# diaoenmao/Multimodal-Controller-for-Generative-Models

Hardware: AMD Instinct MI355X
Metric: images/sec (train step) MCGAN CIFAR-10 32x32 (higher is better)
Workload: dtype bf16

## Files before the change

### include/mcgen_hip.h

```cpp
#ifndef MCGEN_HIP_H
#define MCGEN_HIP_H

#include <stdint.h>

#ifdef __cplusplus
extern "C" {
#endif

enum { MCGEN_F32 = 0, MCGEN_BF16 = 1 };

const char* mcgen_last_error(void);
int mcgen_abi_version(void);

typedef struct {
    const void*  x;
    const float* scale;
    const float* shift;
    const float* code;
    const int16_t* cmap;
    int32_t C;
    int32_t ups;
    int32_t relu;
    int32_t ksize;
    int32_t group_n;
// ... 361 lines not shown
int mcgen_cvae_enc_dembed(const float* part, const float* w, float* de, int N, int H, int C, int Cin, int Cimg, int E,
                          void* stream);
int mcgen_cvae_latent_fwd(const void* ml, int ldm, const float* eps, const float* w, const int64_t* label, float* mu,
                          float* logvar, void* zrow, float* kl, float* kld, int dtype, int N, int L, int E, int M, int Cp,
                          void* stream);
int mcgen_cvae_latent_bwd(const void* dzrow, int ldz, const float* mu, const float* logvar, const float* eps, float inv_numel,
                          void* dml, float* de, int dtype, int N, int L, int E, int Cq, void* stream);

int mcgen_cglow_prior(const float* b_p, const float* s_p, const float* w_e, const float* b_e, const float* s_e,
                      const int64_t* label, void* out, int dtype, int N, int HW, int C2, int M, int Cp, void* stream);
int mcgen_cglow_prior_bwd(const void* dprior, const float* b_p, const float* s_p, const float* w_e, const float* b_e,
                          const float* s_e, const int64_t* label, float* workspace, float* db_p, float* ds_p, float* dw_p,
                          int64_t dw_p_elems, float* dw_e, float* db_e, float* ds_e, int dtype, int N, int HW, int C2, int M,
                          int Cp, void* stream);

#ifdef __cplusplus
}
#endif
#endif
```

### multimodal-controller-for-generative-models_amd/csrc/small_ops.hip

```cpp
#include "mcgen_common.h"
#include <string.h>

static thread_local char g_err[512] = "";
int mcgen_fail(const char* fmt, ...) {
    va_list ap; va_start(ap, fmt); vsnprintf(g_err, sizeof(g_err), fmt, ap); va_end(ap);
    return 1;
}
extern "C" const char* mcgen_last_error(void) { return g_err; }
extern "C" int mcgen_abi_version(void) { return 9; }

namespace {

inline int grid_for(size_t n, int block = 256, int cap = 4096) {
    size_t b = (n + block - 1) / block; if (b < 1) b = 1; if (b > (size_t)cap) b = cap; return (int)b;
}
#define STREAM(s) reinterpret_cast<hipStream_t>(s)

template <typename T> __device__ __forceinline__ float ldf(const T* p) { return Elem<T>::to_f(*p); }

template <typename T>
__global__ void nchw_to_nhwc_kernel(const float* __restrict__ src, T* __restrict__ dst, int N, int C, int HW, int Cp) {
    const size_t total = (size_t)N * HW * Cp;
    for (size_t i = blockIdx.x * (size_t)blockDim.x + threadIdx.x; i < total; i += (size_t)gridDim.x * blockDim.x) {
        const int c = (int)(i % Cp); const size_t pix = i / Cp;
// ... 100 lines not shown
__device__ __forceinline__ void prep_weight_body(const mcgen_prep_t& d, const float* __restrict__ sigma_base) {
    const int KS = d.ksize, Cout = d.Cout, Cin = d.Cin, transpose = d.transpose, row_perm = d.row_perm;
    const float* __restrict__ w = d.w;
    T* __restrict__ img = reinterpret_cast<T*>(d.image);
    const int ntap = KS * KS;
    if (d.layout == 1) {
        const int cow = (Cout + 15) / 16 * 16, krows = (Cin + 7) / 8 * 8 + 1;
        const size_t totalk = (size_t)ntap * krows * cow;
        const float sck = (d.sigma_idx >= 0) ? d.wscale / sigma_base[d.sigma_idx] : d.wscale;
        for (size_t i = blockIdx.x * (size_t)blockDim.x + threadIdx.x; i < totalk; i += (size_t)gridDim.x * blockDim.x) {
            const int co = (int)(i % cow); size_t t = i / cow;
            const int k = (int)(t % krows); const int tap = (int)(t / krows);
            float v = 0.f;
            if (co < Cout && k < Cin) v = w[((size_t)co * Cin + k) * ntap + tap] * sck;
            img[i] = Elem<T>::from_f(v);
        }
        return;
    }
    const int16_t* __restrict__ kmap = transpose ? nullptr : d.kmap;
    const int rows = transpose ? Cin : Cout, kdim = kmap ? d.kcount : (transpose ? Cout : Cin);
    const int rows_w = (rows + 15) / 16 * 16;
    const int nchunk = (((kdim + 7) / 8 * 8) + MCGEN_CK - 1) / MCGEN_CK;
    const float sc = (d.sigma_idx >= 0) ? d.wscale / sigma_base[d.sigma_idx] : d.wscale;
    const int16_t* __restrict__ rmap = transpose ? nullptr : d.rmap;
    __shared__ __attribute__((aligned(16))) T stage[9][8 * MCGEN_CK];
    const int rgroups = rows_w / 8;
    const int groups = nchunk * rgroups;
    const int r8 = threadIdx.x >> 5, col = threadIdx.x & 31;
    constexpr int UPT = 8 * MCGEN_CK * (int)sizeof(T) / 16;
    for (int gi = blockIdx.x; gi < groups; gi += gridDim.x) {
// ... 1509 lines not shown
```

### multimodal-controller-for-generative-models_amd/gan_engine.py

```python
from __future__ import annotations

from typing import Dict, List, Optional

import torch
import torch.nn as nn

from . import ops
from ._tuning import flag as _flag
from .ops import Seg

Tensor = torch.Tensor


def _bump(t: Tensor):
    torch.autograd.graph.increment_version(t)


class FlatState:

    def __init__(self, tensors: List[Tensor]):
        self.tensors = tensors
        self.flat: Optional[Tensor] = None
        self.offsets: List[int] = []
        self._index = {id(t): i for i, t in enumerate(tensors)}
# ... 48 lines not shown
_PM_MAX_MODES = 16
class Nhwc:
    __slots__ = ('t', 'c')

    def __init__(self, t: Tensor, c: int):
        self.t, self.c = t, c

    @property
    def shape(self):
        n, h, w, _ = self.t.shape
        return torch.Size((n, self.c, h, w))


_SN_SNAP = _flag('MCGEN_SN_SNAP', '1') != '0'
_D0_FUSE = _flag('MCGEN_D0_FUSE', '1') != '0'
_BN_PAR = _flag('MCGEN_BN_PAR', '1') != '0'
_pending_counters: Dict[int, List[Tensor]] = {}
_pending_running: List = []


def _flush_counters():
    for k, ts in _pending_counters.items():
        if ts:
            torch._foreach_add_(ts, k)
    _pending_counters.clear()
    if _pending_running:
        ops.bn_running_batch(_pending_running)
        _pending_running.clear()


# ... 486 lines not shown
        red.__exit__(None, None, None)
        yield (0, off_cut if (cut > 0 and _BUCKETS and split) else gflat.numel(), True)


class _SNConv:

    def __init__(self, module: nn.Module, idx: int):
        self.m = module
        self.idx = idx
        w = module.weight_orig
        self.cout, self.cin = w.shape[0], w.shape[1]
        self.ks = w.shape[2] if w.dim() == 4 else 1


class DiscriminatorEngine:
    def __init__(self, dis, dtype: torch.dtype = torch.float32):
        self.dis = dis
        self.dtype = dtype
        blocks = list(dis.blocks.children())
        self.res = [b for b in blocks if hasattr(b, 'mc_1')]
        t = len(self.res)
        self.tail_mc, self.tail_lin = blocks[t + 1], blocks[t + 3].module
        self.sn: List[_SNConv] = []
        for m in dis.modules():
            if hasattr(m, 'weight_orig'):
                self.sn.append(_SNConv(m, len(self.sn)))
        self.sn_of = {s.m: s for s in self.sn}
        params = list(dis.parameters())
        sn_w = {id(s.m.weight_orig) for s in self.sn}
        self.plain = [p for p in params if id(p) not in sn_w]
# ... 35 lines not shown
            self.img[name] = t
            return t

        def cat(name, a: _SNConv, b: _SNConv, transpose):
            na = ops.weight_image_elems(a.cout, a.cin, a.ks, transpose)
            nb = ops.weight_image_elems(b.cout, b.cin, b.ks, transpose)
            t = torch.empty(na + nb, dtype=dt, device=dev)
            self.img[name] = t
            return t[:na], t[na:]

        fwd, bwd = [], []
        W = lambda s: s.m.weight_orig.detach()
        b0 = self.res[0]
        c1m, c2m, scm = (self.sn_of[b0.conv[0].module], self.sn_of[b0.conv[3].module], self.sn_of[b0.shortcut[0].module])
        fwd.append((W(c1m), img('0.c1', c1m, False), False, 1, c1m.idx, 1.0))
        if _D0_FUSE:
            ta, tb = cat('0.c2s', c2m, scm, False)
            fwd += [(W(c2m), ta, False, 1, c2m.idx, 1.0), (W(scm), tb, False, 1, scm.idx, 1.0)]
        else:
            fwd += [(W(scm), img('0.sc', scm, False), False, 1, scm.idx, 1.0),
                    (W(c2m), img('0.c2', c2m, False), False, 1, c2m.idx, 1.0)]
        bwd.append((W(c2m), img('0.c2t', c2m, True), True, 1, c2m.idx, 0.25))
        ta, tb = cat('0.dimg', c1m, scm, True)
        bwd += [(W(c1m), ta, True, 1, c1m.idx, 1.0), (W(scm), tb, True, 1, scm.idx, 0.25)]
        for i, b in enumerate(self.res[1:], start=1):
            c1m, c2m = self.sn_of[b.conv[2].module], self.sn_of[b.conv[5].module]
            has_sc, pooled = len(b.shortcut) > 0, len(b.conv) == 7
            a = 0.25 if pooled else 1.0
            fwd.append((W(c1m), img(f'{i}.c1', c1m, False), False, 1, c1m.idx, 1.0))
            if has_sc:
                scm = self.sn_of[b.shortcut[1].module]
                ta, tb = cat(f'{i}.c2s', c2m, scm, False)
                fwd += [(W(c2m), ta, False, 1, c2m.idx, 1.0), (W(scm), tb, False, 1, scm.idx, 1.0)]
                bwd.append((W(scm), img(f'{i}.sct', scm, True), True, 1, scm.idx, a))
            else:
                fwd.append((W(c2m), img(f'{i}.c2', c2m, False), False, 1, c2m.idx, 1.0))
            bwd += [(W(c2m), img(f'{i}.c2t', c2m, True), True, 1, c2m.idx, a),
                    (W(c1m), img(f'{i}.c1t', c1m, True), True, 1, c1m.idx, 1.0)]
        self._prep_fwd, self._prep_bwd = ops.PrepBatch(fwd, dt), ops.PrepBatch(bwd, dt)
        self._prep_all = ops.PrepBatch(fwd + bwd, dt)
        self._bwd_sigma = None

    def _ensure_preps(self):
        if self._prep_fwd is None or self._prep_fwd.dtype != self.dtype or not self._prep_fwd.valid():
            self._build_preps()

    def _power_iters(self, rounds: int, train: bool):
        fp, fuv = self._ensure_flat()
        nsn = len(self.sn)
        if train and _SN_ROUNDS and not _SN_FUSED and rounds >= int(_flag('MCGEN_SN_ROUNDS_MIN', '1')):
            sigma, snap = ops.sn_power_iter_rounds(fp, fuv, self._layers_dev, nsn, rounds,
                                                   max(s.cout for s in self.sn), max(s.cin * s.ks * s.ks for s in self.sn))
            for s in self.sn:
                _bump(s.m.weight_u); _bump(s.m.weight_v)
            self._sn_ratio = sigma[rounds] if rounds >= 2 else None
            return [(sigma[r], snap[r]) for r in range(rounds)]
        self._sn_ratio = None
        if not _SN_FUSED:
            out = []
# ... 66 lines not shown
            uses = [(None, c1m.idx), (None, scm.idx), (0, c2m.idx)]
            for i, b in enumerate(self.res[1:], start=1):
                c1m, c2m = self.sn_of[b.conv[2].module], self.sn_of[b.conv[5].module]
                uses += [(2 * i - 1, c1m.idx), (2 * i, c2m.idx)]
                if len(b.shortcut) > 0:
                    uses.append((2 * i - 1, self.sn_of[b.shortcut[1].module].idx))
            uses.append((len(self._codes.mcs) - 1, self.sn_of[self.tail_lin].idx))
            self._uses = uses
            self._use_idx = {}
        return self._uses

    def _forward_body(self, x_nchw: Tensor, ctx, code_of, tail_loss: Optional[str] = None):
        dt = self.dtype
        n = x_nchw.shape[0]
        sigma = ctx['sigma']
        self._ensure_preps()
        prep = self._prep_all if ctx.get('train', True) else self._prep_fwd
        job = ctx.pop('codes_job', None)
        if job is not None:
            cb, label, reps, scale, n_half, sink = job
            sink(ops.prep_and_codes(prep, sigma, cb, label, reps, scale, n_half))
        else:
            prep.run(sigma)
        if ctx.get('train', True):
            self._bwd_sigma = sigma
        I = self.img
        img = x_nchw.t if isinstance(x_nchw, Nhwc) else ops.to_nhwc(x_nchw.detach().contiguous(), dt)
        if img.dtype != dt:
            raise RuntimeError(f'Nhwc input is {img.dtype}, the engine computes in {dt}')
        ctx['img'], ctx['nhwc'] = img, isinstance(x_nchw, Nhwc)
        b0 = self.res[0]
        c1m, c2m, scm = (self.sn_of[b0.conv[0].module], self.sn_of[b0.conv[3].module], self.sn_of[b0.shortcut[0].module])
        co = c1m.cout
        c1, _ = ops.conv_fused([Seg(img, code=code_of(None, c1m.idx))], I['0.c1'], co, bias=c1m.m.bias)
        code = code_of(0, c2m.idx)
        if _D0_FUSE:
            y, _ = ops.conv_fused([Seg(c1, code=code, relu=True), Seg(img, ksize=1, code=code_of(None, scm.idx))], I['0.c2s'], co,
                                  bias=c2m.m.bias, bias2=scm.m.bias, pool=True, alpha=0.25)
        else:
            sc, _ = ops.conv_fused([Seg(img, ksize=1, code=code_of(None, scm.idx))], I['0.sc'], co, bias=scm.m.bias, pool=True, alpha=0.25)
            y, _ = ops.conv_fused([Seg(c1, code=code, relu=True)], I['0.c2'], co, bias=c2m.m.bias, pool=True, alpha=0.25, res=sc)
        ctx['blocks'].append({'c1': c1, 'code': code})
        x = y
        for i, b in enumerate(self.res[1:], start=1):
            c1m, c2m = self.sn_of[b.conv[2].module], self.sn_of[b.conv[5].module]
            has_sc = len(b.shortcut) > 0
            pooled = len(b.conv) == 7
            code1, code2 = code_of(2 * i - 1, c1m.idx), code_of(2 * i, c2m.idx)
            code1s = None
            c1, _ = ops.conv_fused([Seg(x, code=code1, relu=True)], I[f'{i}.c1'], c1m.cout, bias=c1m.m.bias)
            if has_sc:
                scm = self.sn_of[b.shortcut[1].module]
                code1s = code_of(2 * i - 1, scm.idx)
# ... 152 lines not shown
                dy, _ = ops.conv_fused([Seg(dc1)], I[f'{bi}.c1t'], c1m.cin, ocode=code1, gate_x=x, res=res)
                if want_w and bi == cut and _BUCKETS and split:
                    red.__exit__(None, None, None)
                    fix(bk['hi'], bk['i_cut'])
                    if _BUCKETS and split:
                        yield (bk['off_cut'], fp.numel(), False)
                    red = ops.deferred_reduces()
                    red.__enter__()
            b0, bc = self.res[0], ctx['blocks'][0]
            c1m, c2m, scm = (self.sn_of[b0.conv[0].module], self.sn_of[b0.conv[3].module], self.sn_of[b0.shortcut[0].module])
            c1, code, img = bc['c1'], bc['code'], ctx['img']
            if want_w:
                wgrad_all(lambda sl: Seg(c1[sl], code=U(0, sl), relu=True), dy, c2m.cout, c2m.cin, c2m.m.weight_orig,
                          c2m.m.bias, scm.m.bias, dy_ups=True, alpha=0.25)
                wgrad_all(lambda sl: Seg(img[sl], ksize=1), dy, scm.cout, scm.cin, scm.m.weight_orig, dy_ups=True, alpha=0.25)
            dc1, _ = ops.conv_fused([Seg(dy, ups=True)], I['0.c2t'], c2m.cin, ocode=code, gate_x=c1)
            if want_w:
                wgrad_all(lambda sl: Seg(img[sl]), dc1, c1m.cout, c1m.cin, c1m.m.weight_orig, c1m.m.bias)
            dimg = None
            if need_input_grad:
                if pair is not None:
                    raise RuntimeError('input gradients of a paired pass are not needed by the D update and not built')
                dimg_t, _ = ops.conv_fused([Seg(dc1), Seg(dy, ksize=1, ups=True)], I['0.dimg'], c1m.cin, cy=img.shape[-1])
                dimg = Nhwc(dimg_t, c1m.cin) if ctx.get('nhwc') else ops.to_nchw(dimg_t, c1m.cin)
        except BaseException as e:
            red.__exit__(type(e), e, None)
            raise
        red.__exit__(None, None, None)
        if want_w:
            if defer_fix and pair is not None and not (_BUCKETS and split) and not accumulate:
                self.pending_fix = {'g0': passes[0][1], 'g1': passes[1][1], 'uv0': uv, 'uv1': pair['uv2'], 'sigma0': sigma,
# ... 8 lines not shown
```

### multimodal-controller-for-generative-models_amd/ops.py

```python
from __future__ import annotations

import ctypes as C
import os as _os
from dataclasses import dataclass
from typing import NamedTuple, Optional, Sequence, Tuple

import torch

from . import _lib
from ._lib import check
from ._tuning import flag as _flag

Tensor = torch.Tensor


def _dt(dtype: torch.dtype) -> int:
    if dtype == torch.float32:
        return _lib.F32
    if dtype == torch.bfloat16:
        return _lib.BF16
    raise _lib.McgenError(f'unsupported compute dtype {dtype}')


def _stream() -> int:
# ... 251 lines not shown
    cout, cin = w.shape[0], w.shape[1]
    ks = w.shape[2] if w.dim() == 4 else 1
    n = weight_image_k_elems(cout, cin, ks)
    if out is None:
        out = torch.empty(n, dtype=dtype, device=w.device)
    assert out.numel() == n and out.dtype == dtype
    check(_lib.load().mcgen_prep_weight_k(_f32(w.contiguous()), _p(out), _dt(dtype), cout, cin, ks, _f32(sigma), float(wscale), _stream()),
          'prep_weight_k')
    return out


def weight_image_elems(cout: int, cin: int, ksize: int, transpose: bool = False) -> int:
    return int(_lib.load().mcgen_weight_image_elems(cout, cin, ksize, int(transpose)))


def prep_weight(w: Tensor, dtype: torch.dtype, transpose: bool = False, row_perm: int = 1,
                sigma: Optional[Tensor] = None, wscale: float = 1.0, out: Optional[Tensor] = None) -> Tensor:
    cout, cin = w.shape[0], w.shape[1]
    ks = w.shape[2] if w.dim() == 4 else 1
    n = weight_image_elems(cout, cin, ks, transpose)
    if out is None:
        out = torch.empty(n, dtype=dtype, device=w.device)
    assert out.numel() == n and out.dtype == dtype
    check(_lib.load().mcgen_prep_weight(_f32(w), _p(out), _dt(dtype), cout, cin, ks, int(transpose), row_perm,
                                        _f32(sigma), float(wscale), _stream()), 'prep_weight')
    return out


def conv_fused(segs: Sequence[Seg], wimg: Tensor, cout: int, *, bias: Optional[Tensor] = None, bias2: Optional[Tensor] = None,
               pool: bool = False, alpha: float = 1.0, res: Optional[Tensor] = None,
               ocode: Optional[Tensor] = None, gate_x: Optional[Tensor] = None,
               gscale: Optional[Tensor] = None, gshift: Optional[Tensor] = None,
               gmean: Optional[Tensor] = None, grstd: Optional[Tensor] = None,
               tanh: bool = False, stats_mode: int = 0, cy: Optional[int] = None,
               out: Optional[Tensor] = None, kmajor: int = 0, ycmap: Optional[Tensor] = None,
               y_group: int = 0, wsel: Optional[Tensor] = None, order: Optional[Tensor] = None,
               yperm: Optional[Tensor] = None) -> Tuple[Tensor, Optional[Tensor]]:
    s0 = segs[0]
    n = s0.x.shape[0]
    h = s0.x.shape[1] * (2 if s0.ups else 1)
    w = s0.x.shape[2] * (2 if s0.ups else 1)
    dtype = s0.x.dtype
    cy = cy or pad8(cout)
    ho, wo = (h // 2, w // 2) if pool else (h, w)
    p = _lib.Conv()
    p.nseg = len(segs)
    for i, s in enumerate(segs):
        if s.x.dtype != dtype:
            raise _lib.McgenError('all segments must share the compute dtype')
        hs = s.x.shape[1] * (2 if s.ups else 1)
        if hs != h or s.x.shape[0] != n:
            raise _lib.McgenError('segments disagree on the convolution resolution')
        s.fill(p.seg[i])
    if wimg.dtype != dtype:
        raise _lib.McgenError(f'weight image dtype {wimg.dtype} != activation dtype {dtype}')
    if kmajor:
        need = sum(s.ksize * s.ksize * ((s.cw or s.x.shape[-1]) + 1) for s in segs) * pad16(cout)
    else:
        need = sum(((s.x.shape[-1] + 31) // 32) * s.ksize * s.ksize for s in segs) * pad16(cout) * 32
    if wsel is not None:
        if wsel.dtype != torch.int32 or wsel.numel() != n or (order is not None and (order.dtype != torch.int32 or order.numel() != n)):
            raise _lib.McgenError('wsel / order must be int32 [N]')
        if wimg.numel() % need:
            raise _lib.McgenError(f'weight sets: {wimg.numel()} elements are not a multiple of one image ({need})')
    elif order is not None:
        raise _lib.McgenError('order comes with wsel')
    elif wimg.numel() != need:
        raise _lib.McgenError(f'weight image has {wimg.numel()} elements, the segments need {need}')
    y = out if out is not None else torch.empty((n, ho, wo, cy), dtype=dtype, device=s0.x.device)
    if y_group:
        if out is None or tuple(y.shape) != (2 * n, ho, wo, cy) or y.dtype != dtype or not y.is_contiguous():
# ... 21 lines not shown
        if wsel is None or yperm.dtype != torch.int16 or yperm.dim() != 2 or yperm.shape[0] * need != wimg.numel() or not yperm.is_contiguous():
            raise _lib.McgenError('yperm must be a contiguous int16 [sets, stride] table that comes with wsel')
        p.yperm, p.yperm_stride = _p(yperm), yperm.shape[1]
    p.ycmap, p.ycmap_stride = None, 0
    if ycmap is not None:
        if ycmap.dtype != torch.int16 or tuple(ycmap.shape) != (n, cmap_stride(pad8(cout))):
            raise _lib.McgenError(f'ycmap must be int16 {(n, cmap_stride(pad8(cout)))}')
        p.ycmap, p.ycmap_stride = _p(ycmap), ycmap.shape[1]
    stats = None
    lib = _lib.load()
    plan = _conv_plan(p, dtype)
    if stats_mode:
        stats = torch.empty((plan.m_tiles, 2, pad16(cout) if (ycmap is not None or yperm is not None) else cy), dtype=torch.float32, device=y.device)
        p.stats = _p(stats)
    kflops = 2.0 * n * h * w * cout * sum(s.ksize * s.ksize * s.x.shape[-1] for s in segs)

    def _name():
        base = f'conv_fused<{"bf16" if dtype == torch.bfloat16 else "f32"},{plan.bm},{plan.bn}{(",mc", ",gk")[kmajor - 1] if kmajor else ""}>'
        if plan.form:
            base = ('conv_skinny<bf16>', 'conv_smap<bf16>', 'conv_px1<bf16>', 'conv_c8<bf16>', 'conv_head<bf16>')[plan.form - 1]
        if _PROF_SHAPES:
            base += f' N{n} {h}x{w} ' + '+'.join(f'{s.x.shape[-1]}k{s.ksize}' for s in segs) + f'->{cout}' + \
                ('g' if gate_x is not None else '') + ('p' if pool else '') + (f's{stats_mode}' if stats_mode else '')
        return base
    if TILE_LOG is not None:
        bm, bn = C.c_int(plan.bm), C.c_int(plan.bn)
        if plan.form:
            check(lib.mcgen_conv_tile(C.byref(p), _dt(dtype), C.byref(bm), C.byref(bn)), 'conv_tile')
        TILE_LOG.append((bm.value, bn.value))
    if FORM_LOG is not None:
        FORM_LOG.append(kmajor)
    if KERNEL_LOG is not None:
        KERNEL_LOG.append(int(plan.form))
    _timed(_name, kflops, lambda: check(lib.mcgen_conv_fused(C.byref(p), _dt(dtype), _stream()), 'conv_fused'),
           lambda: _nbytes(wimg, y, res, gate_x, *[s.x for s in segs]))
    return y, stats


MULTI_LOG = None
WGRAD_LOG = None
BATCH_LOG = None
_deferred = None
_MULTI = _flag('MCGEN_WGRAD_MULTI', '1') != '0'
_BATCH = _flag('MCGEN_WGRAD_BATCH', '1') != '0'
_WG_GROUP_MIN = 1 << 30 if _flag('MCGEN_WGRAD_GROUP', '1') == '0' else 4
_WG_MAX_SPLITS = int(_flag('MCGEN_WGRAD_MAX_SPLITS', '128'))
_WG_TARGET = int(_flag('MCGEN_WGRAD_TARGET', '256'))
_WG_W1 = float(_flag('MCGEN_WG_W1', '0.55'))
_WG_FIX = float(_flag('MCGEN_WG_FIX', '5'))
# ... 506 lines not shown
                                 weight_decay, _p(step), _stream()), 'adam')


def _struct_table(arr, device) -> Tensor:
    return torch.frombuffer(bytearray(bytes(arr)), dtype=torch.uint8).to(device)


class PrepBatch:

    def __init__(self, jobs, dtype: torch.dtype):
        self.dtype = dtype
        self.jobs = jobs
        arr = (_lib.Prep * len(jobs))()
        for d, job in zip(arr, jobs):
            w, img, transpose, row_perm, sidx, wscale = job[:6]
            kmajor = bool(job[6]) if len(job) > 6 else False
            kmap, kcount = (job[7], int(job[8])) if len(job) > 8 and job[7] is not None else (None, 0)
            rmap = job[9] if len(job) > 9 else None
            cout, cin = w.shape[0], w.shape[1]
            ks = w.shape[2] if w.dim() == 4 else 1
            if kmap is not None:
                assert not kmajor and not transpose and row_perm == 1 and kmap.dtype == torch.int16 and kmap.numel() >= kcount
                want = weight_image_elems(cout, kcount, ks, False)
            else:
                want = weight_image_k_elems(cout, cin, ks) if kmajor else weight_image_elems(cout, cin, ks, transpose)
            assert img.numel() == want and img.dtype == dtype and not (kmajor and (transpose or row_perm != 1))
            d.w, d.image = _f32(w), _p(img)
            d.Cout, d.Cin, d.ksize, d.transpose, d.row_perm, d.sigma_idx = cout, cin, ks, int(transpose), row_perm, sidx
            d.wscale, d.layout = float(wscale), int(kmajor)
            d.kmap, d.kcount = _p(kmap), kcount
            if rmap is not None:
                assert not kmajor and not transpose and row_perm == 1 and rmap.dtype == torch.int16 and rmap.numel() >= cout and rmap.is_contiguous()
            d.rmap = _p(rmap)
        self.key = tuple((w.data_ptr(), img.data_ptr()) for w, img, *_ in jobs)
        self.table = _struct_table(arr, jobs[0][0].device)
        self.n = len(jobs)

    def valid(self) -> bool:
        return self.key == tuple((w.data_ptr(), img.data_ptr()) for w, img, *_ in self.jobs)

    def run(self, sigma: Optional[Tensor] = None):
        check(_lib.load().mcgen_prep_weight_batch(_p(self.table), self.n, _f32(sigma), _dt(self.dtype), _stream()),
              'prep_weight_batch')

# ... 810 lines not shown
```

Baseline: 17750.

## Add folded 4x4 kernels for discriminator block0 pooled conv and its backward

Adds specialized HIP kernels for the first discriminator residual block at 32x32. The forward kernel folds the 3x3 conv plus 2x2 average pool into a 16-tap stride-2 conv with the 1x1 shortcut fused in. The backward kernel folds the upsample plus transposed 3x3 conv into four phase-wise 2x2 convs. Both use LDS windows, an async weight ring fed by global_load_lds, and MFMA. New weight-image layouts (2 and 3) are prepared for them, so the pool and upsample no longer waste FLOPs on a full-resolution conv. The cost is a narrow shape guard, a large LDS footprint with one block per CU, and extra prep work.

```diff
diff --git a/include/mcgen_hip.h b/include/mcgen_hip.h
--- a/include/mcgen_hip.h
+++ b/include/mcgen_hip.h
@@ -399,6 +399,13 @@
                           int64_t dw_p_elems, float* dw_e, float* db_e, float* ds_e, int dtype, int N, int HW, int C2, int M,
                           int Cp, void* stream);
 
+int mcgen_conv_fold_fwd_ok(const mcgen_conv_t* p, int dtype);
+int mcgen_conv_fold_fwd(const mcgen_conv_t* p, int dtype, void* stream);
+int mcgen_conv_fold_bwd_ok(const mcgen_conv_t* p, int dtype);
+int mcgen_conv_fold_bwd(const mcgen_conv_t* p, int dtype, void* stream);
+int mcgen_conv_fold_bn(const mcgen_conv_t* p);
+int64_t mcgen_fold_image_elems(int Cout, int Cin, int transpose, int shortcut);
+
 #ifdef __cplusplus
 }
 #endif
diff --git a/multimodal-controller-for-generative-models_amd/csrc/conv_fold.hip b/multimodal-controller-for-generative-models_amd/csrc/conv_fold.hip
--- /dev/null
+++ b/multimodal-controller-for-generative-models_amd/csrc/conv_fold.hip
@@ -0,0 +1,382 @@
+#include "conv_tile.h"
+
+namespace {
+
+constexpr int FD_NT = 512;
+constexpr int FD_WN = 2, FD_FM = 4;
+constexpr int FD_BROW = MCGEN_CK * 2;
+constexpr int FD_RB = 3, FD_DIST = 2;
+constexpr int FD_AP = 96;
+constexpr int FD_COLS = 17, FD_ROWS = 34;
+constexpr int FD_PLANE = FD_ROWS * FD_COLS * FD_AP;
+constexpr int FD_WIN = 2 * FD_PLANE;
+constexpr int FD_TAPS = 16;
+constexpr int FB_PIX = 18 * 18, FB_PB = 256;
+constexpr int FB_WIN = FB_PIX * FB_PB;
+
+template <int BN> struct FdCfg {
+    static constexpr int FN = BN / FD_WN / 16;
+    static constexpr int SLOT = BN * FD_BROW, KB = SLOT / 1024, RING = FD_RB * SLOT;
+    static constexpr int EP = BN + 4;
+    static constexpr int CH = BN / 8, PROWS = FD_NT / CH;
+    static constexpr int FWD_EPI = 256 * EP * 4;
+    static constexpr int FWD_LDS = (FD_WIN + RING) > FWD_EPI ? (FD_WIN + RING) : FWD_EPI;
+    static constexpr int BWD_EPI = 64 * EP * 4;
+    static constexpr int BWD_LDS = FB_WIN + RING + BWD_EPI;
+    static_assert(FWD_LDS <= 160 * 1024 && BWD_LDS <= 160 * 1024, "LDS");
+};
+
+template <int BN>
+struct FdRing {
+    using G = FdCfg<BN>;
+    int d_src;
+    int w_row_off[G::FN];
+    __device__ __forceinline__ void setup(int wave, int lane, int wn, int row0) {
+        const int row = wave * 16 + (lane >> 2), pu = lane & 3;
+        d_src = (row0 + row) * FD_BROW + ((pu ^ (3 * ((row >> 3) & 1))) << 4);
+        const int l15 = lane & 15, lg = lane >> 4;
+#pragma unroll
+        for (int fn = 0; fn < G::FN; ++fn) {
+            const int r = wn * (BN / FD_WN) + fn * 16 + l15;
+            w_row_off[fn] = r * FD_BROW + ((lg ^ (3 * ((r >> 3) & 1))) << 4);
+        }
+    }
+    __device__ __forceinline__ void dma(const char* wblock, char* ring, int slot, int wave) const {
+        if (wave < G::KB)
+            __builtin_amdgcn_global_load_lds((const __attribute__((address_space(1))) void*)(wblock + d_src),
+                                             (__attribute__((address_space(3))) void*)(ring + slot * G::SLOT + wave * 1024), 16, 0, 0);
+    }
+};
+
+static __device__ __forceinline__ void fd_wait_tap(bool more) {
+    if (more) asm volatile("s_waitcnt vmcnt(1)" ::: "memory");
+    else asm volatile("s_waitcnt vmcnt(0)" ::: "memory");
+    asm volatile("s_waitcnt lgkmcnt(0)" ::: "memory");
+    __builtin_amdgcn_s_barrier();
+}
+
+template <int BN>
+__global__ __launch_bounds__(FD_NT, 1)
+void conv_fold_fwd_kernel(const mcgen_conv_t p) {
+    using G = FdCfg<BN>;
+    constexpr int FN = G::FN, FM = FD_FM;
+    extern __shared__ __attribute__((aligned(16))) char smem[];
+    char* const win = smem;
+    char* const ring = smem + FD_WIN;
+    const int tid = threadIdx.x, lane = tid & 63;
+    const int wave = __builtin_amdgcn_readfirstlane(tid >> 6);
+    const int wm = wave >> 1, wn = wave & 1;
+    const int l15 = lane & 15, lg = lane >> 4;
+    const int n = blockIdx.x, cout0 = blockIdx.y * BN;
+    const mcgen_seg_t& s0 = p.seg[0];
+    const int C = s0.C, nchunk = C / MCGEN_CK, total = nchunk * FD_TAPS;
+    const float* anyf = reinterpret_cast<const float*>(p.w);
+    const char* wimg = reinterpret_cast<const char*>(p.w);
+    const size_t wblock = (size_t)p.Cout_w * FD_BROW;
+
+    const int unit = tid & 3, px0 = tid >> 2;
+    const int wc0 = (px0 & 31) + 1;
+    const int lds0 = (wc0 & 1) * FD_PLANE + (((px0 >> 5) + 1) * FD_COLS + (wc0 >> 1)) * FD_AP + unit * 16;
+    const bf16_t* xs = reinterpret_cast<const bf16_t*>(s0.x) + ((size_t)n * 1024 + px0) * C + unit * 8;
+    u32x4 raw[8];
+    float cd[8];
+    auto load_raw = [&](int q) {
+#pragma unroll
+        for (int k = 0; k < 8; ++k) raw[k] = *reinterpret_cast<const u32x4*>(xs + (size_t)k * 128 * C + q * MCGEN_CK);
+        load8f(s0.code ? s0.code + (size_t)n * C + q * MCGEN_CK + unit * 8 : anyf, cd);
+    };
+    load_raw(0);
+
+    bf16x8 sx[FM], sw[FN];
+    float cd1[8];
+    const bool has_sc = p.nseg == 2;
+    if (has_sc) {
+        const bf16_t* x1 = reinterpret_cast<const bf16_t*>(p.seg[1].x) + (size_t)n * 1024 * 8;
+#pragma unroll
+        for (int fm = 0; fm < FM; ++fm)
+            sx[fm] = *reinterpret_cast<const bf16x8*>(x1 + ((2 * (wm * 4 + fm) + (lg >> 1)) * 32 + 2 * l15 + (lg & 1)) * 8);
+        const bf16_t* w1 = reinterpret_cast<const bf16_t*>(wimg + (size_t)total * wblock);
+#pragma unroll
+        for (int fn = 0; fn < FN; ++fn)
+            sw[fn] = *reinterpret_cast<const bf16x8*>(w1 + (size_t)(cout0 + wn * (BN / FD_WN) + fn * 16 + l15) * MCGEN_CK + lg * 8);
+        load8f(p.seg[1].code ? p.seg[1].code + (size_t)n * 8 : anyf, cd1);
+    }
+    asm volatile("" ::: "memory");
+
+    FdRing<BN> rg;
+    rg.setup(wave, lane, wn, cout0);
+    rg.dma(wimg, ring, 0, wave);
+    rg.dma(wimg + wblock, ring, 1, wave);
+
+    for (int i = tid; i < FD_WIN / 16; i += FD_NT) reinterpret_cast<u32x4*>(win)[i] = u32x4{0u, 0u, 0u, 0u};
+
+    f32x4 acc[FN][FM];
+#pragma unroll
+    for (int i = 0; i < FN; ++i)
+#pragma unroll
+        for (int j = 0; j < FM; ++j) acc[i][j] = f32x4{0.f, 0.f, 0.f, 0.f};
+    int a_base[FM];
+#pragma unroll
+    for (int fm = 0; fm < FM; ++fm) a_base[fm] = (2 * (wm * 4 + fm) * FD_COLS + l15) * FD_AP + lg * 16;
+    const float relu_lo = s0.relu ? 0.f : -__builtin_inff();
+
+    int blk = 0;
+#pragma unroll 1
+    for (int q = 0; q < nchunk; ++q) {
+        asm volatile("s_waitcnt lgkmcnt(0)" ::: "memory");
+        __builtin_amdgcn_s_barrier();
+#pragma unroll
+        for (int k = 0; k < 8; ++k) {
+            union { bf16x8 h; u32x4 w; } o;
+#pragma unroll
+            for (int e = 0; e < 4; ++e) {
+                const float v0 = fmaxf(__uint_as_float(raw[k][e] << 16), relu_lo), v1 = fmaxf(__uint_as_float(raw[k][e] & 0xffff0000u), relu_lo);
+                o.h[2 * e] = (bf16_t)(s0.code ? v0 * cd[2 * e] : v0);
+                o.h[2 * e + 1] = (bf16_t)(s0.code ? v1 * cd[2 * e + 1] : v1);
+            }
+            *reinterpret_cast<u32x4*>(win + lds0 + k * (4 * FD_COLS * FD_AP)) = o.w;
+        }
+#pragma unroll 1
+        for (int tap = 0; tap < FD_TAPS; ++tap) {
+            fd_wait_tap(blk + 1 < total);
+            if (tap == FD_TAPS / 2 && q + 1 < nchunk) {
+                load_raw(q + 1);
+                asm volatile("" ::: "memory");
+            }
+            if (blk + FD_DIST < total) rg.dma(wimg + (size_t)(blk + FD_DIST) * wblock, ring, (blk + FD_DIST) % FD_RB, wave);
+            const int a = tap >> 2, b = tap & 3;
+            const char* wa = win + (b & 1) * FD_PLANE + (a * FD_COLS + (b >> 1)) * FD_AP;
+            const char* wb = ring + (blk % FD_RB) * G::SLOT;
+            bf16x8 af[FM], wf[FN];
+#pragma unroll
+            for (int fm = 0; fm < FM; ++fm) af[fm] = *reinterpret_cast<const bf16x8*>(wa + a_base[fm]);
+#pragma unroll
+            for (int fn = 0; fn < FN; ++fn) wf[fn] = *reinterpret_cast<const bf16x8*>(wb + rg.w_row_off[fn]);
+#pragma unroll
+            for (int fn = 0; fn < FN; ++fn)
+#pragma unroll
+                for (int fm = 0; fm < FM; ++fm) acc[fn][fm] = __builtin_amdgcn_mfma_f32_16x16x32_bf16(wf[fn], af[fm], acc[fn][fm], 0, 0, 0);
+            ++blk;
+        }
+    }
+    if (has_sc) {
+#pragma unroll
+        for (int fm = 0; fm < FM; ++fm) {
+            if (p.seg[1].code) {
+#pragma unroll
+                for (int e = 0; e < 8; ++e) sx[fm][e] = (bf16_t)((float)sx[fm][e] * cd1[e]);
+            }
+#pragma unroll
+            for (int fn = 0; fn < FN; ++fn) acc[fn][fm] = __builtin_amdgcn_mfma_f32_16x16x32_bf16(sw[fn], sx[fm], acc[fn][fm], 0, 0, 0);
+        }
+    }
+    asm volatile("s_waitcnt vmcnt(0) lgkmcnt(0)" ::: "memory");
+    __syncthreads();
+    float* epi = reinterpret_cast<float*>(smem);
+#pragma unroll
+    for (int fn = 0; fn < FN; ++fn)
+#pragma unroll
+        for (int fm = 0; fm < FM; ++fm)
+            *reinterpret_cast<f32x4*>(epi + (wm * 64 + fm * 16 + l15) * G::EP + wn * (BN / FD_WN) + fn * 16 + lg * 4) = acc[fn][fm];
+    const int ch = tid % G::CH, prow = tid / G::CH;
+    const int co = cout0 + ch * 8;
+    float bs[8], b2[8];
+    load8f(p.bias ? p.bias + co : anyf, bs);
+    load8f(p.bias2 ? p.bias2 + co : anyf, b2);
+#pragma unroll
+    for (int e = 0; e < 8; ++e) bs[e] = (p.bias ? bs[e] : 0.f) + (p.bias2 ? b2[e] : 0.f);
+    __syncthreads();
+    bf16_t* yb = reinterpret_cast<bf16_t*>(p.y) + (size_t)n * 256 * p.Cy + co;
+#pragma unroll 4
+    for (int mo = prow; mo < 256; mo += G::PROWS) {
+        const f32x4 a = *reinterpret_cast<const f32x4*>(epi + mo * G::EP + ch * 8), b = *reinterpret_cast<const f32x4*>(epi + mo * G::EP + ch * 8 + 4);
+        float v[8];
+#pragma unroll
+        for (int e = 0; e < 4; ++e) { v[e] = fmaf(a[e], p.alpha, bs[e]); v[4 + e] = fmaf(b[e], p.alpha, bs[4 + e]); }
+        Elem<bf16_t>::store8(yb + (size_t)mo * p.Cy, v);
+    }
+}
+
+static __device__ __forceinline__ int fb_off(int wr, int wc, int unit) { return (wr * 18 + wc) * FB_PB + ((unit ^ (wc & 15)) << 4); }
+
+template <int BN>
+__global__ __launch_bounds__(FD_NT, 1)
+void conv_fold_bwd_kernel(const mcgen_conv_t p) {
+    using G = FdCfg<BN>;
+    constexpr int FN = G::FN, FM = FD_FM;
+    constexpr int NCH = FB_PB / FD_BROW;
+    constexpr int TOTAL = 4 * NCH * 4;
+    extern __shared__ __attribute__((aligned(16))) char smem[];
+    char* const win = smem;
+    char* const ring = smem + FB_WIN;
+    float* const epi = reinterpret_cast<float*>(smem + FB_WIN + G::RING);
+    const int tid = threadIdx.x, lane = tid & 63;
+    const int wave = __builtin_amdgcn_readfirstlane(tid >> 6);
+    const int wm = wave >> 1, wn = wave & 1;
+    const int l15 = lane & 15, lg = lane >> 4;
+    const int n = blockIdx.x, c0 = blockIdx.y * BN;
+    const float* anyf = reinterpret_cast<const float*>(p.w);
+    const char* wimg = reinterpret_cast<const char*>(p.w);
+    const size_t wblock = (size_t)p.Cout_w * FD_BROW;
+
+    u32x4 raw[8];
+    {
+        const bf16_t* dy = reinterpret_cast<const bf16_t*>(p.seg[0].x) + (size_t)n * 256 * 128 + (size_t)(tid >> 4) * 128 + (tid & 15) * 8;
+#pragma unroll
+        for (int k = 0; k < 8; ++k) raw[k] = *reinterpret_cast<const u32x4*>(dy + (size_t)k * 32 * 128);
+    }
+    asm volatile("" ::: "memory");
+    auto block_of = [&](int s) { return ((s >> 2) & (NCH - 1)) * 16 + (s / (4 * NCH)) * 4 + (s & 3); };
+    FdRing<BN> rg;
+    rg.setup(wave, lane, wn, c0);
+    rg.dma(wimg + (size_t)block_of(0) * wblock, ring, 0, wave);
+    rg.dma(wimg + (size_t)block_of(1) * wblock, ring, 1, wave);
+
+    for (int i = tid; i < FB_WIN / 16; i += FD_NT) reinterpret_cast<u32x4*>(win)[i] = u32x4{0u, 0u, 0u, 0u};
+    __syncthreads();
+#pragma unroll
+    for (int k = 0; k < 8; ++k) {
+        const int px = (tid >> 4) + 32 * k;
+        *reinterpret_cast<u32x4*>(win + fb_off((px >> 4) + 1, (px & 15) + 1, tid & 15)) = raw[k];
+    }
+
+    const int ch = tid % G::CH, prow = tid / G::CH;
+    const int co = c0 + ch * 8;
+    float bs[8], oc[8];
+    load8f(p.bias ? p.bias + co : anyf, bs);
+    load8f(p.ocode ? p.ocode + (size_t)n * p.Cout + co : anyf, oc);
+#pragma unroll
+    for (int e = 0; e < 8; ++e) { bs[e] = p.bias ? bs[e] : 0.f; oc[e] = p.ocode ? oc[e] : 1.f; }
+    const bf16_t* gx = p.gate_x ? reinterpret_cast<const bf16_t*>(p.gate_x) : reinterpret_cast<const bf16_t*>(p.w);
+    bf16_t* yb = reinterpret_cast<bf16_t*>(p.y);
+    asm volatile("" ::: "memory");
+
+    int s = 0;
+#pragma unroll 1
+    for (int P = 0; P < 4; ++P) {
+        const int py = P >> 1, px = P & 1;
+        f32x4 acc[FN][FM];
+#pragma unroll
+        for (int i = 0; i < FN; ++i)
+#pragma unroll
+            for (int j = 0; j < FM; ++j) acc[i][j] = f32x4{0.f, 0.f, 0.f, 0.f};
+#pragma unroll 1
+        for (int q = 0; q < NCH; ++q) {
+#pragma unroll 1
+            for (int uv = 0; uv < 4; ++uv) {
+                fd_wait_tap(s + 1 < TOTAL);
+                if (s + FD_DIST < TOTAL) rg.dma(wimg + (size_t)block_of(s + FD_DIST) * wblock, ring, (s + FD_DIST) % FD_RB, wave);
+                const int wc = l15 + px + (uv & 1);
+                const char* wb = ring + (s % FD_RB) * G::SLOT;
+                bf16x8 af[FM], wf[FN];
+#pragma unroll
+                for (int fm = 0; fm < FM; ++fm) af[fm] = *reinterpret_cast<const bf16x8*>(win + fb_off(wm * 4 + fm + py + (uv >> 1), wc, q * 4 + lg));
+#pragma unroll
+                for (int fn = 0; fn < FN; ++fn) wf[fn] = *reinterpret_cast<const bf16x8*>(wb + rg.w_row_off[fn]);
+#pragma unroll
+                for (int fn = 0; fn < FN; ++fn)
+#pragma unroll
+                    for (int fm = 0; fm < FM; ++fm) acc[fn][fm] = __builtin_amdgcn_mfma_f32_16x16x32_bf16(wf[fn], af[fm], acc[fn][fm], 0, 0, 0);
+                ++s;
+            }
+        }
+#pragma unroll 1
+        for (int pass = 0; pass < 4; ++pass) {
+            if (pass > 0 || P > 0) __syncthreads();
+            if (wm == pass) {
+#pragma unroll
+                for (int fn = 0; fn < FN; ++fn)
+#pragma unroll
+                    for (int fm = 0; fm < FM; ++fm)
+                        *reinterpret_cast<f32x4*>(epi + (fm * 16 + l15) * G::EP + wn * (BN / FD_WN) + fn * 16 + lg * 4) = acc[fn][fm];
+            }
+            __syncthreads();
+#pragma unroll
+            for (int mo = prow; mo < 64; mo += G::PROWS) {
+                const int Y = pass * 4 + (mo >> 4), X = mo & 15;
+                const size_t off = (((size_t)n * 32 + 2 * Y + py) * 32 + 2 * X + px) * p.Cy + co;
+                const u32x4 g = *reinterpret_cast<const u32x4*>(gx + (p.gate_x ? off : 0));
+                const f32x4 a = *reinterpret_cast<const f32x4*>(epi + mo * G::EP + ch * 8), b = *reinterpret_cast<const f32x4*>(epi + mo * G::EP + ch * 8 + 4);
+                float v[8];
+#pragma unroll
+                for (int e = 0; e < 4; ++e) { v[e] = fmaf(a[e], p.alpha, bs[e]) * oc[e]; v[4 + e] = fmaf(b[e], p.alpha, bs[4 + e]) * oc[4 + e]; }
+                if (p.gate_x) {
+#pragma unroll
+                    for (int e = 0; e < 4; ++e) {
+                        if (!(__uint_as_float(g[e] << 16) > 0.f)) v[2 * e] = 0.f;
+                        if (!(__uint_as_float(g[e] & 0xffff0000u) > 0.f)) v[2 * e + 1] = 0.f;
+                    }
+                }
+                Elem<bf16_t>::store8(yb + off, v);
+            }
+        }
+    }
+}
+
+static bool fold_common(const mcgen_conv_t* p, int dtype) {
+    if (!p || dtype != MCGEN_BF16 || p->w_layout != 0 || p->N < 1 || p->H != 32 || p->W != 32) return false;
+    if (p->Cout % 64 || p->Cout_w != p->Cout || p->Cy != p->Cout) return false;
+    if (p->res || p->gscale || p->tanh_out || p->stats_mode || p->ycmap || p->y_group || p->wsel || p->order || p->yperm) return false;
+    const mcgen_seg_t& g = p->seg[0];
+    return g.ksize == 3 && !g.scale && !g.cmap && g.group_n == 0 && g.C > 0;
+}
+
+static bool fwd_ok(const mcgen_conv_t* p, int dtype) {
+    if (!fold_common(p, dtype) || !p->pool || p->ocode || p->gate_x || p->nseg < 1 || p->nseg > 2) return false;
+    if (p->seg[0].ups || p->seg[0].C % MCGEN_CK) return false;
+    if (p->nseg == 2) {
+        const mcgen_seg_t& g = p->seg[1];
+        if (g.ksize != 1 || g.C != 8 || g.ups || g.relu || g.scale || g.cmap || g.group_n) return false;
+    }
+    return true;
+}
+
+static bool bwd_ok(const mcgen_conv_t* p, int dtype) {
+    if (!fold_common(p, dtype) || p->pool || p->nseg != 1 || p->bias2) return false;
+    const mcgen_seg_t& g = p->seg[0];
+    return g.ups == 1 && g.C == FB_PB / 2 && !g.relu && !g.code;
+}
+
+static int fold_bn(const mcgen_conv_t* p) { return (p->Cout % 128 == 0 && (long)p->N * (p->Cout / 128) >= 256) ? 128 : 64; }
+
+template <typename K>
+static int fold_launch(K k, const char* who, int lds, int bn, const mcgen_conv_t* p, hipStream_t st, bool* raised) {
+    if (!*raised) {
+        hipError_t e = hipFuncSetAttribute(reinterpret_cast<const void*>(k), hipFuncAttributeMaxDynamicSharedMemorySize, lds);
+        if (e != hipSuccess) return mcgen_fail("%s: cannot raise LDS limit: %s", who, hipGetErrorString(e));
+        *raised = true;
+    }
+    hipLaunchKernelGGL(k, dim3(p->N, p->Cout / bn), dim3(FD_NT), lds, st, *p);
+    MCGEN_LAUNCH_CHECK(who);
+    return 0;
+}
+
+}
+
+extern "C" int mcgen_conv_fold_fwd_ok(const mcgen_conv_t* p, int dtype) { return fwd_ok(p, dtype) ? 1 : 0; }
+extern "C" int mcgen_conv_fold_bwd_ok(const mcgen_conv_t* p, int dtype) { return bwd_ok(p, dtype) ? 1 : 0; }
+extern "C" int mcgen_conv_fold_bn(const mcgen_conv_t* p) { return p ? fold_bn(p) : 0; }
+
+extern "C" int64_t mcgen_fold_image_elems(int Cout, int Cin, int transpose, int shortcut) {
+    const int rows = transpose ? Cin : Cout, kdim = transpose ? Cout : Cin;
+    const int64_t rows_w = round_up(rows, 16);
+    return (int64_t)round_up(kdim, MCGEN_CK) / MCGEN_CK * FD_TAPS * rows_w * MCGEN_CK + (shortcut ? rows_w * MCGEN_CK : 0);
+}
+
+extern "C" int mcgen_conv_fold_fwd(const mcgen_conv_t* p, int dtype, void* stream) {
+    MCGEN_CHECK(fwd_ok(p, dtype), "conv_fold_fwd: not a pooled 3x3 launch this kernel takes (bf16, 32x32, Cin %% 32 == 0, Cout %% 64 == 0, plain epilogue)");
+    MCGEN_CHECK(p->w && p->y && p->seg[0].x && (p->nseg == 1 || p->seg[1].x), "conv_fold_fwd: missing buffer");
+    static bool r128 = false, r64 = false;
+    hipStream_t st = reinterpret_cast<hipStream_t>(stream);
+    if (fold_bn(p) == 128) return fold_launch(conv_fold_fwd_kernel<128>, "conv_fold_fwd", FdCfg<128>::FWD_LDS, 128, p, st, &r128);
+    return fold_launch(conv_fold_fwd_kernel<64>, "conv_fold_fwd", FdCfg<64>::FWD_LDS, 64, p, st, &r64);
+}
+
+extern "C" int mcgen_conv_fold_bwd(const mcgen_conv_t* p, int dtype, void* stream) {
+    MCGEN_CHECK(bwd_ok(p, dtype), "conv_fold_bwd: not an upsampled-dy 3x3 input gradient this kernel takes (bf16, 32x32, 128 dy channels, Cout %% 64 == 0)");
+    MCGEN_CHECK(p->w && p->y && p->seg[0].x, "conv_fold_bwd: missing buffer");
+    static bool r128 = false, r64 = false;
+    hipStream_t st = reinterpret_cast<hipStream_t>(stream);
+    if (fold_bn(p) == 128) return fold_launch(conv_fold_bwd_kernel<128>, "conv_fold_bwd", FdCfg<128>::BWD_LDS, 128, p, st, &r128);
+    return fold_launch(conv_fold_bwd_kernel<64>, "conv_fold_bwd", FdCfg<64>::BWD_LDS, 64, p, st, &r64);
+}
diff --git a/multimodal-controller-for-generative-models_amd/csrc/small_ops.hip b/multimodal-controller-for-generative-models_amd/csrc/small_ops.hip
--- a/multimodal-controller-for-generative-models_amd/csrc/small_ops.hip
+++ b/multimodal-controller-for-generative-models_amd/csrc/small_ops.hip
@@ -138,6 +138,49 @@
             float v = 0.f;
             if (co < Cout && k < Cin) v = w[((size_t)co * Cin + k) * ntap + tap] * sck;
             img[i] = Elem<T>::from_f(v);
+        }
+        return;
+    }
+    if (d.layout == 2) {
+        const int rows = transpose ? Cin : Cout, kdim = transpose ? Cout : Cin;
+        const int rows_w = (rows + 15) / 16 * 16, nchunk = (kdim + MCGEN_CK - 1) / MCGEN_CK;
+        const size_t totalf = (size_t)nchunk * 16 * rows_w * MCGEN_CK;
+        const float scf = (d.sigma_idx >= 0) ? d.wscale / sigma_base[d.sigma_idx] : d.wscale;
+        for (size_t i = blockIdx.x * (size_t)blockDim.x + threadIdx.x; i < totalf; i += (size_t)gridDim.x * blockDim.x) {
+            const int col = (int)(i % MCGEN_CK); size_t t = i / MCGEN_CK;
+            const int row = (int)(t % rows_w); t /= rows_w;
+            const int tap = (int)(t % 16), k = (int)(t / 16) * MCGEN_CK + col;
+            float v = 0.f;
+            if (row < rows && k < kdim) {
+                const float* src = w + ((size_t)(transpose ? k : row) * Cin + (transpose ? row : k)) * 9;
+                int t0, t1, s0, s1;
+                if (!transpose) {
+                    const int a = tap >> 2, b = tap & 3;
+                    t0 = a > 0 ? a - 1 : 0; t1 = a < 2 ? a : 2; s0 = b > 0 ? b - 1 : 0; s1 = b < 2 ? b : 2;
+                } else {
+                    const int py = tap >> 3, px = (tap >> 2) & 1, u = (tap >> 1) & 1, vv = tap & 1;
+                    t0 = py ? (u ? 0 : 1) : (u ? 0 : 2); t1 = py ? (u ? 0 : 2) : (u ? 1 : 2);
+                    s0 = px ? (vv ? 0 : 1) : (vv ? 0 : 2); s1 = px ? (vv ? 0 : 2) : (vv ? 1 : 2);
+                }
+                bool first = true;
+                for (int tt = t0; tt <= t1; ++tt)
+                    for (int ss = s0; ss <= s1; ++ss) {
+#pragma clang fp contract(off)
+                        const float term = src[tt * 3 + ss] * scf;
+                        v = first ? term : v + term;
+                        first = false;
+                    }
+            }
+            img[i] = Elem<T>::from_f(v);
+        }
+        return;
+    }
+    if (d.layout == 3) {
+        const int rows_w = (Cout + 15) / 16 * 16;
+        const float scs = (d.sigma_idx >= 0) ? d.wscale / sigma_base[d.sigma_idx] : d.wscale;
+        for (size_t i = blockIdx.x * (size_t)blockDim.x + threadIdx.x; i < (size_t)rows_w * MCGEN_CK; i += (size_t)gridDim.x * blockDim.x) {
+            const int col = (int)(i % MCGEN_CK), row = (int)(i / MCGEN_CK), ci = col & 7;
+            img[i] = Elem<T>::from_f((row < Cout && ci < Cin) ? w[(size_t)row * Cin + ci] * scs : 0.f);
         }
         return;
     }
diff --git a/multimodal-controller-for-generative-models_amd/gan_engine.py b/multimodal-controller-for-generative-models_amd/gan_engine.py
--- a/multimodal-controller-for-generative-models_amd/gan_engine.py
+++ b/multimodal-controller-for-generative-models_amd/gan_engine.py
@@ -86,6 +86,7 @@
 
 _SN_SNAP = _flag('MCGEN_SN_SNAP', '1') != '0'
 _D0_FUSE = _flag('MCGEN_D0_FUSE', '1') != '0'
+_D_FOLD = _flag('MCGEN_D_FOLD', '0') != '0'
 _BN_PAR = _flag('MCGEN_BN_PAR', '1') != '0'
 _pending_counters: Dict[int, List[Tensor]] = {}
 _pending_running: List = []
@@ -602,6 +603,9 @@
 
 
 class DiscriminatorEngine:
+    _fold = False
+    _fold_built = False
+
     def __init__(self, dis, dtype: torch.dtype = torch.float32):
         self.dis = dis
         self.dtype = dtype
@@ -667,13 +671,23 @@
         b0 = self.res[0]
         c1m, c2m, scm = (self.sn_of[b0.conv[0].module], self.sn_of[b0.conv[3].module], self.sn_of[b0.shortcut[0].module])
         fwd.append((W(c1m), img('0.c1', c1m, False), False, 1, c1m.idx, 1.0))
-        if _D0_FUSE:
+        self._fold_built = self._fold
+        if self._fold:
+            na = ops.fold_image_elems(c2m.cout, c2m.cin, False)
+            t = torch.empty(ops.fold_image_elems(c2m.cout, c2m.cin, False, True), dtype=dt, device=dev)
+            self.img['0.c2s'] = t
+            fwd += [(W(c2m), t[:na], False, 1, c2m.idx, 1.0, 2), (W(scm), t[na:], False, 1, scm.idx, 1.0, 3)]
+            t = torch.empty(ops.fold_image_elems(c2m.cout, c2m.cin, True), dtype=dt, device=dev)
+            self.img['0.c2t'] = t
+            bwd.append((W(c2m), t, True, 1, c2m.idx, 0.25, 2))
+        elif _D0_FUSE:
             ta, tb = cat('0.c2s', c2m, scm, False)
             fwd += [(W(c2m), ta, False, 1, c2m.idx, 1.0), (W(scm), tb, False, 1, scm.idx, 1.0)]
         else:
             fwd += [(W(scm), img('0.sc', scm, False), False, 1, scm.idx, 1.0),
                     (W(c2m), img('0.c2', c2m, False), False, 1, c2m.idx, 1.0)]
-        bwd.append((W(c2m), img('0.c2t', c2m, True), True, 1, c2m.idx, 0.25))
+        if not self._fold:
+            bwd.append((W(c2m), img('0.c2t', c2m, True), True, 1, c2m.idx, 0.25))
         ta, tb = cat('0.dimg', c1m, scm, True)
         bwd += [(W(c1m), ta, True, 1, c1m.idx, 1.0), (W(scm), tb, True, 1, scm.idx, 0.25)]
         for i, b in enumerate(self.res[1:], start=1):
@@ -694,8 +708,15 @@
         self._prep_all = ops.PrepBatch(fwd + bwd, dt)
         self._bwd_sigma = None
 
+    def _fold_ok(self, h: int, w: int) -> bool:
+        b0 = self.res[0]
+        c2m, scm = self.sn_of[b0.conv[3].module], self.sn_of[b0.shortcut[0].module]
+        return (_D_FOLD and _D0_FUSE and self.dtype == torch.bfloat16 and h == 32 and w == 32 and scm.cin <= 8
+                and c2m.cin % 32 == 0 and c2m.cin % 64 == 0 and c2m.cout == 128)
+
     def _ensure_preps(self):
-        if self._prep_fwd is None or self._prep_fwd.dtype != self.dtype or not self._prep_fwd.valid():
+        if self._prep_fwd is None or self._prep_fwd.dtype != self.dtype or not self._prep_fwd.valid() \
+                or self._fold_built != self._fold:
             self._build_preps()
 
     def _power_iters(self, rounds: int, train: bool):
@@ -792,6 +813,7 @@
         dt = self.dtype
         n = x_nchw.shape[0]
         sigma = ctx['sigma']
+        self._fold = ctx['fold'] = self._fold_ok(x_nchw.shape[2], x_nchw.shape[3])
         self._ensure_preps()
         prep = self._prep_all if ctx.get('train', True) else self._prep_fwd
         job = ctx.pop('codes_job', None)
@@ -814,7 +836,7 @@
         code = code_of(0, c2m.idx)
         if _D0_FUSE:
             y, _ = ops.conv_fused([Seg(c1, code=code, relu=True), Seg(img, ksize=1, code=code_of(None, scm.idx))], I['0.c2s'], co,
-                                  bias=c2m.m.bias, bias2=scm.m.bias, pool=True, alpha=0.25)
+                                  bias=c2m.m.bias, bias2=scm.m.bias, pool=True, alpha=0.25, fold=self._fold)
         else:
             sc, _ = ops.conv_fused([Seg(img, ksize=1, code=code_of(None, scm.idx))], I['0.sc'], co, bias=scm.m.bias, pool=True, alpha=0.25)
             y, _ = ops.conv_fused([Seg(c1, code=code, relu=True)], I['0.c2'], co, bias=c2m.m.bias, pool=True, alpha=0.25, res=sc)
@@ -997,7 +1019,7 @@
                 wgrad_all(lambda sl: Seg(c1[sl], code=U(0, sl), relu=True), dy, c2m.cout, c2m.cin, c2m.m.weight_orig,
                           c2m.m.bias, scm.m.bias, dy_ups=True, alpha=0.25)
                 wgrad_all(lambda sl: Seg(img[sl], ksize=1), dy, scm.cout, scm.cin, scm.m.weight_orig, dy_ups=True, alpha=0.25)
-            dc1, _ = ops.conv_fused([Seg(dy, ups=True)], I['0.c2t'], c2m.cin, ocode=code, gate_x=c1)
+            dc1, _ = ops.conv_fused([Seg(dy, ups=True)], I['0.c2t'], c2m.cin, ocode=code, gate_x=c1, fold=ctx.get('fold', False))
             if want_w:
                 wgrad_all(lambda sl: Seg(img[sl]), dc1, c1m.cout, c1m.cin, c1m.m.weight_orig, c1m.m.bias)
             dimg = None
diff --git a/multimodal-controller-for-generative-models_amd/ops.py b/multimodal-controller-for-generative-models_amd/ops.py
--- a/multimodal-controller-for-generative-models_amd/ops.py
+++ b/multimodal-controller-for-generative-models_amd/ops.py
@@ -289,6 +289,10 @@
     return int(_lib.load().mcgen_weight_image_elems(cout, cin, ksize, int(transpose)))
 
 
+def fold_image_elems(cout: int, cin: int, transpose: bool = False, shortcut: bool = False) -> int:
+    return int(_lib.load().mcgen_fold_image_elems(cout, cin, int(transpose), int(shortcut)))
+
+
 def prep_weight(w: Tensor, dtype: torch.dtype, transpose: bool = False, row_perm: int = 1,
                 sigma: Optional[Tensor] = None, wscale: float = 1.0, out: Optional[Tensor] = None) -> Tensor:
     cout, cin = w.shape[0], w.shape[1]
@@ -310,7 +314,7 @@
                tanh: bool = False, stats_mode: int = 0, cy: Optional[int] = None,
                out: Optional[Tensor] = None, kmajor: int = 0, ycmap: Optional[Tensor] = None,
                y_group: int = 0, wsel: Optional[Tensor] = None, order: Optional[Tensor] = None,
-               yperm: Optional[Tensor] = None) -> Tuple[Tensor, Optional[Tensor]]:
+               yperm: Optional[Tensor] = None, fold: bool = False) -> Tuple[Tensor, Optional[Tensor]]:
     s0 = segs[0]
     n = s0.x.shape[0]
     h = s0.x.shape[1] * (2 if s0.ups else 1)
@@ -329,7 +333,10 @@
         s.fill(p.seg[i])
     if wimg.dtype != dtype:
         raise _lib.McgenError(f'weight image dtype {wimg.dtype} != activation dtype {dtype}')
-    if kmajor:
+    fold_bwd = fold and not pool
+    if fold:
+        need = fold_image_elems(s0.x.shape[-1], cout, True) if fold_bwd else fold_image_elems(cout, s0.x.shape[-1], False, len(segs) == 2)
+    elif kmajor:
         need = sum(s.ksize * s.ksize * ((s.cw or s.x.shape[-1]) + 1) for s in segs) * pad16(cout)
     else:
         need = sum(((s.x.shape[-1] + 31) // 32) * s.ksize * s.ksize for s in segs) * pad16(cout) * 32
@@ -381,8 +388,16 @@
         stats = torch.empty((plan.m_tiles, 2, pad16(cout) if (ycmap is not None or yperm is not None) else cy), dtype=torch.float32, device=y.device)
         p.stats = _p(stats)
     kflops = 2.0 * n * h * w * cout * sum(s.ksize * s.ksize * s.x.shape[-1] for s in segs)
+    if fold:
+        ok = lib.mcgen_conv_fold_bwd_ok if fold_bwd else lib.mcgen_conv_fold_fwd_ok
+        if not ok(C.byref(p), _dt(dtype)):
+            raise _lib.McgenError('conv_fused(fold=True): the folded kernels do not take this launch')
+        kflops = 2.0 * n * (h // 2) * (w // 2) * cout * (16 * s0.x.shape[-1] + (32 if len(segs) == 2 else 0))
 
     def _name():
+        if fold:
+            return f'conv_fold_{"bwd" if fold_bwd else "fwd"}<bf16,{lib.mcgen_conv_fold_bn(C.byref(p))}>' + \
+                (f' N{n} {h}x{w} {s0.x.shape[-1]}->{cout}' if _PROF_SHAPES else '')
         base = f'conv_fused<{"bf16" if dtype == torch.bfloat16 else "f32"},{plan.bm},{plan.bn}{(",mc", ",gk")[kmajor - 1] if kmajor else ""}>'
         if plan.form:
             base = ('conv_skinny<bf16>', 'conv_smap<bf16>', 'conv_px1<bf16>', 'conv_c8<bf16>', 'conv_head<bf16>')[plan.form - 1]
@@ -399,7 +414,8 @@
         FORM_LOG.append(kmajor)
     if KERNEL_LOG is not None:
         KERNEL_LOG.append(int(plan.form))
-    _timed(_name, kflops, lambda: check(lib.mcgen_conv_fused(C.byref(p), _dt(dtype), _stream()), 'conv_fused'),
+    entry = (lib.mcgen_conv_fold_bwd if fold_bwd else lib.mcgen_conv_fold_fwd) if fold else lib.mcgen_conv_fused
+    _timed(_name, kflops, lambda: check(entry(C.byref(p), _dt(dtype), _stream()), 'conv_fused'),
            lambda: _nbytes(wimg, y, res, gate_x, *[s.x for s in segs]))
     return y, stats
 
@@ -936,7 +952,8 @@
         arr = (_lib.Prep * len(jobs))()
         for d, job in zip(arr, jobs):
             w, img, transpose, row_perm, sidx, wscale = job[:6]
-            kmajor = bool(job[6]) if len(job) > 6 else False
+            layout = int(job[6]) if len(job) > 6 else 0
+            kmajor = layout == 1
             kmap, kcount = (job[7], int(job[8])) if len(job) > 8 and job[7] is not None else (None, 0)
             rmap = job[9] if len(job) > 9 else None
             cout, cin = w.shape[0], w.shape[1]
@@ -944,12 +961,18 @@
             if kmap is not None:
                 assert not kmajor and not transpose and row_perm == 1 and kmap.dtype == torch.int16 and kmap.numel() >= kcount
                 want = weight_image_elems(cout, kcount, ks, False)
+            elif layout == 2:
+                assert ks == 3 and row_perm == 1
+                want = fold_image_elems(cout, cin, bool(transpose))
+            elif layout == 3:
+                assert ks == 1 and cin <= 8 and not transpose and row_perm == 1
+                want = pad16(cout) * 32
             else:
                 want = weight_image_k_elems(cout, cin, ks) if kmajor else weight_image_elems(cout, cin, ks, transpose)
             assert img.numel() == want and img.dtype == dtype and not (kmajor and (transpose or row_perm != 1))
             d.w, d.image = _f32(w), _p(img)
             d.Cout, d.Cin, d.ksize, d.transpose, d.row_perm, d.sigma_idx = cout, cin, ks, int(transpose), row_perm, sidx
-            d.wscale, d.layout = float(wscale), int(kmajor)
+            d.wscale, d.layout = float(wscale), layout
             d.kmap, d.kcount = _p(kmap), kcount
             if rmap is not None:
                 assert not kmajor and not transpose and row_perm == 1 and rmap.dtype == torch.int16 and rmap.numel() >= cout and rmap.is_contiguous()
```

Result: no change. 17720 (-0.1%).
